# Kyaw-Thiha/animal-vision

Hardware: AMD Instinct MI355X
Metric: megapixels/sec per-frame pipeline (higher is better)
Workload: dtype f16

## Files before the change

animal-vision_amd/csrc/mst_fused.hip:

```cpp
#include <hip/hip_fp16.h>

#include <cstdio>
#include <cstdlib>
#include <cstring>

#include "avx_internal.h"
#include "mst_common.h"
#include "mst_tile_order.h"

namespace {

typedef float float4_t __attribute__((ext_vector_type(4)));
#ifndef AVX_FFN32_GM2
#define AVX_FFN32_GM2 1
#endif
constexpr int kFT = 512;
constexpr int TS = 16;
constexpr int HS = TS + 2;
#ifndef AVX_FFN_TH
#define AVX_FFN_TH 16
#endif
constexpr int kFfnTH = AVX_FFN_TH;
static_assert(kFfnTH == 14 || kFfnTH == 16, "FeedForward tile rows");
constexpr int kFfnNGRP = (HS * (kFfnTH + 2) + 31) / 32;

__device__ __forceinline__ float16_t mfma16(half8_t a, half8_t b, float16_t c) { return __builtin_amdgcn_mfma_f32_32x32x16_f16(a, b, c, 0, 0, 0); }

struct Tile { int x0, y0; long b; };
template <class Walk>
__device__ __forceinline__ Tile tile_at(const Walk& wk, int side_x, int side_y) { return Tile{wk.xi * side_x, wk.yi * side_y, (long)wk.b}; }
int mst_tile_order() {
    const char* e = getenv("AVX_MST_TILE_ORDER");
    return e && !strcmp(e, "raster") ? AVX_TILE_ORDER_RASTER : AVX_TILE_ORDER_XCD;
}

typedef _Float16 half16_t __attribute__((ext_vector_type(16)));
template <bool DWS>
__device__ __forceinline__ float4_t dw_unit(const half8_t (&a)[3], const uint4 (&bq)[3]) {
    float4_t acc = {0.f, 0.f, 0.f, 0.f};
    if constexpr (DWS) {
        const half8_t b0 = __builtin_bit_cast(half8_t, bq[0]), b1 = __builtin_bit_cast(half8_t, bq[1]);
        acc = __builtin_amdgcn_mfma_f32_16x16x32_f16(a[1], __builtin_bit_cast(half8_t, bq[2]), acc, 0, 0, 0);
        acc = __builtin_amdgcn_smfmac_f32_16x16x64_f16(a[0], __builtin_shufflevector(b0, b1, 0, 1, 2, 3, 4, 5, 6, 7, 8, 9, 10, 11, 12, 13, 14, 15), acc,
                                                       (int)__builtin_bit_cast(uint4, a[2]).x, 0, 0);
    } else {
#pragma unroll
        for (int i = 0; i < 3; ++i) acc = __builtin_amdgcn_mfma_f32_16x16x32_f16(a[i], __builtin_bit_cast(half8_t, bq[i]), acc, 0, 0, 0);
    }
    return acc;
}
template <bool DWS>
__device__ __forceinline__ half8_t dw_frag(const uint4* p, int i) {
    if (DWS && i == 2) return __builtin_bit_cast(half8_t, uint4{*reinterpret_cast<const unsigned*>(p), 0u, 0u, 0u});
    return __builtin_bit_cast(half8_t, *p);
}
template <bool MARCH> struct FfnWalk { typedef TileWalk type; };
template <> struct FfnWalk<true> { typedef ColumnWalk type; };
template <int C, int HPASS, int MINW, bool DWM, bool STAMP = false, int NW = 8, bool DWS = false, bool MARCH = false>
__global__ __launch_bounds__(64 * NW, MINW) void k_mst_ffn_fused(const __half* __restrict__ x , const float* __restrict__ gamma, const float* __restrict__ beta,
                                                          float eps, const uint4* __restrict__ w1pack , const __half* __restrict__ taps ,
                                                          const uint4* __restrict__ w2pack , __half* __restrict__ out , int B,
                                                          int H, int W, const uint4* __restrict__ dwpack , unsigned long long* __restrict__ stamps , int order ) {
    constexpr int FTH = MARCH ? 14 : kFfnTH, HSY = FTH + 2, ROW0 = MARCH ? 2 : 0, NHALO = HS * (HSY - ROW0), NGRP = (NHALO + 31) / 32;
    constexpr int HID = 4 * C, NPASS = HID / HPASS, KS1 = C / 16, KS2 = HPASS / 16, NT = C / 32, YPITCH = C * 2 + 16, LNV = C / 16;
    constexpr int HPITCH = HPASS * 2 + 16, RPITCH = (HS * HPITCH + 255) / 256 * 256 , NCT = HPASS / 32;
    static_assert(C == 32 || C == 64 || C == 128, "31-, 62- or 124-channel blocks (stored 32 / 64 / 128 wide)");
    constexpr int NTHR = 64 * NW, NGW = (NGRP + NW - 1) / NW;
    constexpr int NTW = NT / (NW / 8), NOCTW = HPASS / (8 * NW);
    static_assert((NW == 8 || NW == 16) && NT % (NW / 8) == 0 && (!DWM || HPASS % (8 * NW) == 0) && (DWM || NW == 8) && (DWM || !DWS) && (DWM || !MARCH), "wave split");
    constexpr bool PREFETCH = C <= 64;
    extern __shared__ __align__(16) unsigned char smem[];
    unsigned char* yt = smem;
    unsigned char* ht = yt + (size_t)NGRP * 32 * YPITCH;
    __half* tapl = reinterpret_cast<__half*>(ht + (size_t)HSY * RPITCH);
    float* gl = reinterpret_cast<float*>(tapl + (DWM ? 0 : 9 * HID));
    constexpr bool W2LDS = NW == 16;
    uint4* w2l = reinterpret_cast<uint4*>(gl + 2 * C);
    constexpr int NPRIME = 2 * HS, CARRY = NPRIME * HPITCH;
    unsigned char* carry = reinterpret_cast<unsigned char*>(w2l + (W2LDS ? NT * KS2 * 64 : 0));
    const int tid = threadIdx.x, lane = tid & 63, wave = tid >> 6, p = lane & 31, h = lane >> 5;
    unsigned long long seg[8] = {0, 0, 0, 0, 0, 0, 0, 0}, tlast = 0;
// ... 131 lines not shown
                    const float bq = is_pad(i + 1) ? 0.f : __builtin_fmaf(d[i + 1] * rstd, gl[c + 1], gl[C + c + 1]);
                    o[j / 2] = pack_f16(a, bq);
                }
                *reinterpret_cast<uint4*>(dst + 16 * v) = uint4{o[0], o[1], o[2], o[3]};
            }
        }
    };

    const int n0 = (wave / 8) * NTW, w8 = wave % 8;
    half8_t w2f[W2LDS ? 1 : NTW * KS2];
    auto load_w2 = [&](int pass) {
#pragma unroll
        for (int n = 0; n < NTW; ++n)
#pragma unroll
            for (int s = 0; s < KS2; ++s) w2f[n * KS2 + s] = __builtin_bit_cast(half8_t, w2pack[((size_t)(n0 + n) * (HID / 16) + pass * KS2 + s) * 64 + lane]);
    };
    if constexpr (NPASS == 1 && !W2LDS) load_w2(0);
    half8_t w1f[KS1];
    auto load_w1 = [&](int pass) {
#pragma unroll
        for (int s = 0; s < KS1; ++s) w1f[s] = __builtin_bit_cast(half8_t, w1pack[((size_t)(pass * NCT + wave % NCT) * KS1 + s) * 64 + lane]);
    };
    constexpr bool W1AHEAD = DWM && C == 64 && NPASS > 1 && NW == 8;
    static_assert(!(MARCH && W1AHEAD), "the marching form loads W1 at the top of phase 1 (priming replaces the fragments)");
    if constexpr (W1AHEAD) load_w1(0);
    constexpr int NITEM = (NGRP + NW / NCT - 1) / (NW / NCT);
    int p1_g[NITEM], p1_dst[NITEM], p1_dy[NITEM], p1_dx[NITEM];
#pragma unroll
    for (int j = 0; j < NITEM; ++j) {
        const int g = wave / NCT + j * (NW / NCT), q = 32 * g + p, qc = q < NHALO ? q : 0;
        p1_g[j] = g < NGRP ? g : -1;
        p1_dst[j] = (g < NGRP && q < NHALO) ? (ROW0 + qc / HS) * RPITCH + (qc % HS) * HPITCH + 32 * h : -1;
        p1_dy[j] = ROW0 + qc / HS - 1; p1_dx[j] = qc % HS - 1;
    }
    auto p1_item = [&](int g, unsigned char* base, int off, bool masked, int yy, int xx) {
        float16_t d;
#pragma unroll
        for (int v = 0; v < 16; ++v) d[v] = 0.f;
        const unsigned char* ysrc = yt + (size_t)(32 * g + p) * YPITCH + 16 * h;
#pragma unroll
        for (int s = 0; s < KS1; ++s) d = mfma16(w1f[s], __builtin_bit_cast(half8_t, *reinterpret_cast<const uint4*>(ysrc + 32 * s)), d);
        if (off >= 0) {
            unsigned char* dst = base + off;
            uint32_t keep = 0xffffffffu;
            if (masked) keep = (yy >= 0 && yy < H && xx >= 0 && xx < W) ? 0xffffffffu : 0u;
            constexpr int GP1 = (C == 64 && NW == 8) ? 4 : (C == 32 ? 2 : 1);
            unsigned pk[8];
#pragma unroll
// ... 19 lines not shown
        int td = tid;
        asm volatile("" : "+v"(td));
        const int wl = td >> 6, q = 32 * (wl / NCT) + (td & 31), qc = q < NPRIME ? q : 0, yy = t.y0 - 1 + qc / HS, xx = t.x0 - 1 + qc % HS;
        const int off = q < NPRIME ? qc * HPITCH + 32 * ((td >> 5) & 1) + 64 * (wl % NCT) : -1;
        if (g < NGPRIME) {
#pragma unroll 1
            for (int pass = 0; pass < NPASS; ++pass) {
                load_w1(pass);
                p1_item(g, carry + (size_t)pass * CARRY, off, true, yy, xx);
            }
        }
        __syncthreads();
    };
    typename FfnWalk<MARCH>::type ahead;
    if constexpr (MARCH) ahead.init(blockIdx.x, gridDim.x, B, ty, tx);
    else ahead.init(blockIdx.x, gridDim.x, B, ty, tx, order);
    if (!ahead.live) return;
    Tile t = tile_at(ahead, TS, FTH);
    ahead.advance();
    if constexpr (MARCH) prime(t);
    fetch(t);
    __syncthreads();
    layernorm(NGRP);
    for (;;) {
        const bool halo_inside = t.y0 + ROW0 >= 1 && t.y0 + HSY - 1 <= H && t.x0 >= 1 && t.x0 + HS - 1 <= W;
        float16_t D[NTW];
#pragma unroll
        for (int n = 0; n < NTW; ++n)
#pragma unroll
            for (int v = 0; v < 16; ++v) D[n][v] = 0.f;
#pragma unroll 1
        for (int pass = 0; pass < NPASS; ++pass) {
            stamp(pass == 0 ? 7 : 5);
            __syncthreads();
            stamp(0);
            if constexpr (W2LDS)
                for (int i = tid; i < NT * KS2 * 64; i += NTHR) w2l[i] = w2pack[((size_t)(i / (KS2 * 64)) * (HID / 16) + pass * KS2 + (i / 64) % KS2) * 64 + (i & 63)];
            half8_t af[DWM ? NOCTW : 1][3];
            if constexpr (DWM) {
#pragma unroll
                for (int o2 = 0; o2 < NOCTW; ++o2)
#pragma unroll
                    for (int i = 0; i < 3; ++i) af[o2][i] = dw_frag<DWS>(dwpack + ((size_t)(pass * (HPASS / 8) + NW * o2 + wave) * 3 + i) * 64 + lane, i);
            }
            {
                const int ct = wave % NCT;
                if constexpr (!W1AHEAD) load_w1(pass);
                if constexpr (MARCH) {
                    constexpr int NV = NPRIME * (HPASS / 8);
                    static_assert(NV <= NTHR, "one 16-byte piece per thread");
                    int i = tid;
                    asm volatile("" : "+v"(i));
                    if (i < NV) {
                        const int px = i / (HPASS / 8), o = i % (HPASS / 8);
                        *reinterpret_cast<uint4*>(ht + (size_t)(px / HS) * RPITCH + (size_t)(px % HS) * HPITCH + 16 * o) =
                            *reinterpret_cast<const uint4*>(carry + (size_t)pass * CARRY + (size_t)px * HPITCH + 16 * o);
                    }
                }
#pragma unroll
                for (int j = 0; j < NITEM; ++j) {
                    if (p1_g[j] < 0) continue;
                    p1_item(p1_g[j], ht + 64 * ct, p1_dst[j], !halo_inside, t.y0 + p1_dy[j], t.x0 + p1_dx[j]);
                }
            }
            stamp(1);
            __syncthreads();
            stamp(2);
            bool ahead_fetch = ahead.live;
            if constexpr (MARCH) ahead_fetch = ahead_fetch && !ahead.seg;
            if (PREFETCH && pass == NPASS - 1 && ahead_fetch) fetch(tile_at(ahead, TS, FTH));
// ... 93 lines not shown
#pragma unroll
                    for (int j = 0; j < 8; ++j) acc[j] = 0.f;
#pragma unroll
                    for (int tap = 0; tap < 9; ++tap) {
                        const uint4 hv = *reinterpret_cast<const uint4*>(hbase + (size_t)(tap / 3) * RPITCH + (size_t)(tap % 3) * HPITCH + 32 * s);
                        const uint4 wv = *reinterpret_cast<const uint4*>(tbase + (size_t)tap * HID * 2 + 32 * s);
                        fma_mix_lo(acc[0], hv.x, wv.x); fma_mix_hi(acc[1], hv.x, wv.x);
                        fma_mix_lo(acc[2], hv.y, wv.y); fma_mix_hi(acc[3], hv.y, wv.y);
                        fma_mix_lo(acc[4], hv.z, wv.z); fma_mix_hi(acc[5], hv.z, wv.z);
                        fma_mix_lo(acc[6], hv.w, wv.w); fma_mix_hi(acc[7], hv.w, wv.w);
                    }
                    half8_t bf;
#pragma unroll
                    for (int j = 0; j < 8; j += 2) {
                        const float2_t gv = gelu_fast2(float2_t{acc[j], acc[j + 1]});
                        bf[j] = (_Float16)gv.x;
                        bf[j + 1] = (_Float16)gv.y;
                    }
#pragma unroll
                    for (int n = 0; n < NT; ++n)
                        D[n] = mfma16(w2f[n * KS2 + s], bf, D[n]);
                }
            }
        }
        stamp(5);
        {
            const int yo = t.y0 + 2 * w8 + (p >> 4), xo = t.x0 + (p & 15);
            if (2 * w8 < FTH && yo < H && xo < W) {
                const size_t off = ((t.b * H + yo) * (size_t)W + xo) * C + 16 * h + 32 * n0;
#pragma unroll
                for (int n = 0; n < NTW; ++n) {
                    const uint4 xa = reinterpret_cast<const uint4*>(x + off + 32 * n)[0], xb = reinterpret_cast<const uint4*>(x + off + 32 * n)[1];
                    const unsigned xw[8] = {xa.x, xa.y, xa.z, xa.w, xb.x, xb.y, xb.z, xb.w};
                    unsigned ow[8];
#pragma unroll
                    for (int j = 0; j < 8; ++j) {
                        float s0 = D[n][2 * j], s1 = D[n][2 * j + 1];
                        fma_mix_lo(s0, xw[j], 0x3c003c00u); fma_mix_hi(s1, xw[j], 0x3c003c00u);
                        ow[j] = pack_f16(s0, s1);
                    }
                    reinterpret_cast<uint4*>(out + off + 32 * n)[0] = uint4{ow[0], ow[1], ow[2], ow[3]};
                    reinterpret_cast<uint4*>(out + off + 32 * n)[1] = uint4{ow[4], ow[5], ow[6], ow[7]};
                }
            }
        }
        stamp(6);
        if (!ahead.live) break;
        t = tile_at(ahead, TS, FTH);
        bool fetch_now = !PREFETCH;
        if constexpr (MARCH) {
            if (ahead.seg) { prime(t); fetch_now = true; }
        }
        ahead.advance();
        if (fetch_now) fetch(t);
        layernorm(NGRP);
    }
    if constexpr (STAMP) {
        if (lane == 0 && stamps)
#pragma unroll
            for (int k = 0; k < 8; ++k) stamps[((size_t)blockIdx.x * NW + wave) * 8 + k] = seg[k];
    }
}


constexpr int VS = TS + 4, MS = TS + 2;

template <int C, int MINW>
__global__ __launch_bounds__(kFT, MINW) void k_mst_attn_tail(const __half* __restrict__ v , const __half* __restrict__ x ,
                                                             const uint4* __restrict__ mpack , const __half* __restrict__ taps1 ,
                                                             const __half* __restrict__ taps2 , const float* __restrict__ bias ,
                                                             __half* __restrict__ out, int B, int H, int W, const uint4* __restrict__ wvpack ) {
    constexpr int NO = C / 8, NS = C / 16, NT = C / 32, PP = C * 2 + 16;
    constexpr int VRP = (VS * PP + 255) / 256 * 256, MRP = VRP;
    constexpr int NFILL = (VS * VS * NO + kFT - 1) / kFT;
    extern __shared__ __align__(16) unsigned char smem[];
    unsigned char* vt = smem;
    unsigned char* mt = vt + (size_t)VS * VRP;
    const bool fromx = wvpack != nullptr;
// ... 828 lines not shown
}
__device__ __forceinline__ void conv_in_mfma(const unsigned raw[5], half8_t a0, half8_t a1, uint4 o[2]) {
    const float inv255 = 1.0f / 255.0f;
    float v[16];
    v[15] = 0.f;
#pragma unroll
    for (int t = 0; t < 5; ++t)
#pragma unroll
        for (int c = 0; c < 3; ++c) v[3 * t + c] = (float)((raw[t] >> (8 * c)) & 0xffu) * inv255;
    const half8_t b0 = __builtin_bit_cast(half8_t, uint4{pack_f16(v[0], v[1]), pack_f16(v[2], v[3]), pack_f16(v[4], v[5]), pack_f16(v[6], v[7])});
    const half8_t b1 = __builtin_bit_cast(half8_t, uint4{pack_f16(v[8], v[9]), pack_f16(v[10], v[11]), pack_f16(v[12], v[13]), pack_f16(v[14], v[15])});
    float16_t d;
#pragma unroll
    for (int vv = 0; vv < 16; ++vv) d[vv] = 0.f;
    d = mfma16(a0, b0, d);
    d = mfma16(a1, b1, d);
    unsigned q[8];
#pragma unroll
    for (int vv = 0; vv < 8; ++vv) q[vv] = pack_f16(d[2 * vv], d[2 * vv + 1]);
    o[0] = uint4{q[0], q[1], q[2], q[3]};
    o[1] = uint4{q[4], q[5], q[6], q[7]};
}

template <int MINW, bool GRAM, bool SPEC = false, bool CINR = false, bool CINX = false>
__global__ __launch_bounds__(kFT, MINW) void k_mst_conv3x3_lds(const __half* __restrict__ x , const uint4* __restrict__ wpack ,
                                                               const __half* __restrict__ add , __half* __restrict__ out, int B, int H, int W,
                                                               const uint4* __restrict__ wqk , float* __restrict__ partial ,
                                                               const float* __restrict__ specw = nullptr ,
                                                               float* __restrict__ planes = nullptr , SpecStat3* __restrict__ spart = nullptr ,
                                                               int crop_t = 0, int crop_l = 0, int Hc = 0, int Wc = 0, int order = AVX_TILE_ORDER_RASTER ,
                                                               ConvInFrame cf = ConvInFrame{nullptr, 0, 0, 0, 0, 0, 0} , const float* __restrict__ cw = nullptr ) {
    static_assert(!(CINR && CINX), "the frame stands in for the residual or for the input");
    constexpr bool CIN = CINR || CINX;
    constexpr int C = 32, PP = C * 2 + 16, RP = (HS * PP + 255) / 256 * 256, NFILL = CINX ? 1 : (HS * HS * 4 + kFT - 1) / kFT;
    constexpr int SS = HS + 2;
    __shared__ __align__(16) unsigned char xt[HS * RP];
    __shared__ uint4 wl[18 * 64];
    __shared__ uint4 cwl[CIN ? 2 * 64 : 1];
    __shared__ unsigned st[CINX ? SS * SS : 1];
    const int tid = threadIdx.x, lane = tid & 63, wave = tid >> 6, p = lane & 31, h = lane >> 5;
    for (int i = tid; i < 18 * 64; i += kFT) wl[i] = wpack[i];
    if constexpr (CIN) {
        if (tid < 2 * 64) cwl[tid] = __builtin_bit_cast(uint4, conv_in_afrag(cw, lane, wave));
    }
    __shared__ uint4 wq[GRAM ? 4 * 64 : 1];
    float16_t G;
    float nq = 0.f, nk = 0.f;
    if constexpr (GRAM) {
        if (tid < 4 * 64) wq[tid] = wqk[tid];
#pragma unroll
        for (int v = 0; v < 16; ++v) G[v] = 0.f;
    }
    float smn[3] = {3.4e38f, 3.4e38f, 3.4e38f}, smx[3] = {-3.4e38f, -3.4e38f, -3.4e38f};
    double ssum[3] = {0.0, 0.0, 0.0};
    const int tx = (W + TS - 1) / TS, ty = (H + TS - 1) / TS;
    uint4 pre[NFILL];
    unsigned f_rel[NFILL];
#pragma unroll
    for (int k = 0; k < NFILL; ++k) {
        const int it = tid + k * kFT, itc = it < HS * HS * 4 ? it : 0, q = itc >> 2, part = itc & 3;
        f_rel[k] = (unsigned)(((q / HS) * W + q % HS) * C + 8 * part) * 2u;
    }
    auto fetch = [&](const Tile& t) {
        int tq = tid;
// ... 117 lines not shown
                if (add) { ar[0] = reinterpret_cast<const uint4*>(add + off)[0]; ar[1] = reinterpret_cast<const uint4*>(add + off)[1]; }
            }
            float16_t d;
#pragma unroll
            for (int v = 0; v < 16; ++v) d[v] = 0.f;
            const unsigned char* src = xt + (size_t)r * RP + (size_t)c * PP + 16 * h;
#pragma unroll
            for (int tap = 0; tap < 9; ++tap)
#pragma unroll
                for (int s2 = 0; s2 < 2; ++s2)
                    d = mfma16(__builtin_bit_cast(half8_t, wl[(2 * tap + s2) * 64 + lane]), __builtin_bit_cast(half8_t, *reinterpret_cast<const uint4*>(src + (size_t)(tap / 3) * RP + (size_t)(tap % 3) * PP + 32 * s2)), d);
            half8_t o0, o1;
            {
                const half8_t r0 = __builtin_bit_cast(half8_t, ar[0]), r1 = __builtin_bit_cast(half8_t, ar[1]);
#pragma unroll
                for (int v = 0; v < 8; ++v) { o0[v] = (_Float16)(d[v] + (float)r0[v]); o1[v] = (_Float16)(d[8 + v] + (float)r1[v]); }
            }
            if constexpr (SPEC) {
                float a3[3] = {0.f, 0.f, 0.f};
                auto chain = [&]() {
#pragma unroll
                    for (int j = 0; j < 16; ++j) {
                        const float v = (float)(j < 8 ? o0[j] : o1[j - 8]);
                        const float* wb = specw + (16 * h + j) * 4;
#pragma unroll
                        for (int k = 0; k < 3; ++k) a3[k] = __builtin_fmaf(v, wb[k], a3[k]);
                    }
                };
                if (h == 0) chain();
#pragma unroll
                for (int k = 0; k < 3; ++k) { const float lo = __shfl_xor(a3[k], 32); a3[k] = h ? lo : a3[k]; }
                if (h == 1) chain();
                const int yc = yo - crop_t, xc = xo - crop_l;
                if (h == 1 && live && yc >= 0 && yc < Hc && xc >= 0 && xc < Wc) {
#pragma unroll
                    for (int k = 0; k < 3; ++k) {
                        planes[(size_t)k * Hc * Wc + (size_t)yc * Wc + xc] = a3[k];
                        smn[k] = fminf(smn[k], a3[k]); smx[k] = fmaxf(smx[k], a3[k]); ssum[k] += (double)a3[k];
                    }
                }
            } else if (live) {
                reinterpret_cast<uint4*>(out + off)[0] = __builtin_bit_cast(uint4, o0);
                reinterpret_cast<uint4*>(out + off)[1] = __builtin_bit_cast(uint4, o1);
            }
            if constexpr (GRAM) {
                if (!live) { o0 = half8_t{0, 0, 0, 0, 0, 0, 0, 0}; o1 = o0; }
                float16_t dq, dk;
// ... 374 lines not shown
                            const void* w2pack, void* out, int B, int H, int W, int C, void* stream, bool sparse, bool march, int max_workgroups) {
    AVX_REQUIRE(ctx, x && gamma && beta && w1pack && w2pack && out && B > 0 && H > 0 && W > 0, "avx_mst_ffn_fused: NULL pointer or empty tensor");
    AVX_REQUIRE(ctx, C == 32 || C == 64 || C == 128, "avx_mst_ffn_fused: C=%d (32, 64 or 128: 31-channel groups stored 32 wide)", C);
    AVX_REQUIRE(ctx, ((((uintptr_t)x | (uintptr_t)w1pack | (uintptr_t)w2pack | (uintptr_t)out | (uintptr_t)taps_9xhid)) & 15u) == 0,
                "avx_mst_ffn_fused: pointers must be 16-byte aligned");
    AVX_REQUIRE(ctx, x != out, "avx_mst_ffn_fused: neighbouring tiles read each other's halo: the output cannot be the input");
    AVX_HIP(ctx, hipSetDevice(ctx->device));
    hipStream_t s = avx_pick_stream(ctx, stream);
    const int fth = march ? 14 : kFfnTH;
    const long total = (long)B * ((H + fth - 1) / fth) * ((W + TS - 1) / TS);
    const char* hp = getenv("AVX_MST_FFN_HPASS");
    const bool small = C == 32 && (march || !(hp && atoi(hp) == 128));
    const int hpass = (small || C == 128) ? 64 : 128, hpitch = hpass * 2 + 16, rpitch = (HS * hpitch + 255) / 256 * 256;
    const long cap = (long)ctx->num_cus * (small ? 2 : 1);
    const bool nw16 = C == 64 && dwpack && (march || !(getenv("AVX_MST_FFN_NW") && atoi(getenv("AVX_MST_FFN_NW")) == 8));
    const size_t lds = (size_t)(march ? 8 : kFfnNGRP) * 32 * (C * 2 + 16) + (size_t)(fth + 2) * rpitch + (dwpack ? 0 : (size_t)9 * 4 * C * 2) + sizeof(float) * 2 * C +
                       (nw16 ? (size_t)(C / 32) * (hpass / 16) * 1024 : 0) + (march ? (size_t)(4 * C / hpass) * 2 * HS * hpitch : 0);
    AVX_REQUIRE(ctx, total <= 0x7fffffffl, "avx_mst_ffn_fused: 2^31 tiles or more");
    AVX_REQUIRE(ctx, !march || (dwpack && (C == 32 || C == 64)), "avx_mst_ffn_fused: the marching form is built for the matrix-pipe kernels at C = 32 and 64");
    long nwg = total < cap ? total : cap;
    if (max_workgroups > 0 && max_workgroups < nwg) nwg = max_workgroups;
    const dim3 grid((unsigned)nwg);
    const int order = mst_tile_order();
#define AVX_FFN1M(CV, HP, MW, DW, NWV, SP, MR)                                                                                                   \
    {                                                                                                                                            \
        auto k = k_mst_ffn_fused<CV, HP, MW, DW, false, NWV, SP, MR>;                                                                            \
        AVX_HIP(ctx, hipFuncSetAttribute((const void*)k, hipFuncAttributeMaxDynamicSharedMemorySize, (int)lds));                                 \
        hipLaunchKernelGGL(k, grid, dim3(64 * NWV), lds, s, (const __half*)x, gamma, beta, eps, (const uint4*)w1pack, (const __half*)taps_9xhid, \
                           (const uint4*)w2pack, (__half*)out, B, H, W, (const uint4*)dwpack, (unsigned long long*)nullptr, order);              \
    }
#define AVX_FFN1S(CV, HP, MW, DW, NWV, SP) AVX_FFN1M(CV, HP, MW, DW, NWV, SP, false)
#define AVX_FFN1(CV, HP, MW, DW, NWV) AVX_FFN1S(CV, HP, MW, DW, NWV, false)
#define AVX_FFN(CV, HP, MW) { if (dwpack && sparse) AVX_FFN1S(CV, HP, MW, true, 8, true) else if (dwpack) AVX_FFN1(CV, HP, MW, true, 8) else AVX_FFN1(CV, HP, MW, false, 8) }
    if (dwpack && getenv("AVX_FFN_STAMPS") && ((C == 32 && small) || C == 64 || C == 128)) {
        unsigned long long* d_st = nullptr;
        const int nwv = nw16 ? 16 : 8;
        const size_t n = (size_t)grid.x * nwv * 8;
        AVX_HIP(ctx, hipMalloc((void**)&d_st, n * sizeof(unsigned long long)));
#define AVX_FFN_ST2(CV, HP, MW, NWV, SP, MR)                                                                                                     \
    {                                                                                                                                            \
        auto k = k_mst_ffn_fused<CV, HP, MW, true, true, NWV, SP, MR>;                                                                           \
        AVX_HIP(ctx, hipFuncSetAttribute((const void*)k, hipFuncAttributeMaxDynamicSharedMemorySize, (int)lds));                                 \
        hipLaunchKernelGGL(k, grid, dim3(64 * NWV), lds, s, (const __half*)x, gamma, beta, eps, (const uint4*)w1pack, (const __half*)taps_9xhid, \
                           (const uint4*)w2pack, (__half*)out, B, H, W, (const uint4*)dwpack, d_st, order);                                      \
    }
#define AVX_FFN_ST1(CV, HP, MW, NWV, SP) AVX_FFN_ST2(CV, HP, MW, NWV, SP, false)
#define AVX_FFN_ST(CV, HP, MW, NWV) { if (sparse) AVX_FFN_ST1(CV, HP, MW, NWV, true) else AVX_FFN_ST1(CV, HP, MW, NWV, false) }
#define AVX_FFN_STM(CV, HP, MW, NWV) { if (sparse) AVX_FFN_ST2(CV, HP, MW, NWV, true, true) else AVX_FFN_ST2(CV, HP, MW, NWV, false, true) }
        if (march && C == 32) AVX_FFN_STM(32, 64, 4, 8) else if (march) AVX_FFN_STM(64, 128, 1, 16)
        else if (C == 32) AVX_FFN_ST(32, 64, 4, 8) else if (nw16) AVX_FFN_ST(64, 128, 1, 16) else if (C == 64) AVX_FFN_ST(64, 128, 2, 8) else AVX_FFN_ST(128, 64, 2, 8)
#undef AVX_FFN_STM
#undef AVX_FFN_ST
#undef AVX_FFN_ST1
#undef AVX_FFN_ST2
        AVX_HIP(ctx, hipStreamSynchronize(s));
        unsigned long long* h_st = (unsigned long long*)malloc(n * sizeof(unsigned long long));
        AVX_HIP(ctx, hipMemcpy(h_st, d_st, n * sizeof(unsigned long long), hipMemcpyDeviceToHost));
        double tot[8] = {0}, w0[8] = {0}, w7[8] = {0};
        for (size_t i = 0; i < n; ++i) { tot[i & 7] += (double)h_st[i]; if (((i >> 3) % nwv) == 0) w0[i & 7] += (double)h_st[i]; if (((i >> 3) % nwv) == (size_t)nwv - 1) w7[i & 7] += (double)h_st[i]; }
        double all = 0;
        for (int k2 = 0; k2 < 8; ++k2) all += tot[k2];
        fprintf(stderr, "[ffn stamps C=%d%s] %u blocks x %d waves, mean cycles per wave %.0f; share per segment (all waves | first wave | last wave): ", C, march ? " march" : "", grid.x, nwv, all / (grid.x * (double)nwv));
        const char* nm[8] = {"bar1", "phase1", "bar2", "phase2a", "bar3", "phase2b", "epilogue", "ln+fetch"};
        for (int k2 = 0; k2 < 8; ++k2) fprintf(stderr, "%s %.1f%% | %.1f%% | %.1f%%  ", nm[k2], 100 * tot[k2] / all, 100 * w0[k2] * nwv / all, 100 * w7[k2] * nwv / all);
        fprintf(stderr, "\n");
        free(h_st);
        (void)hipFree(d_st);
    } else if (march && C == 32 && sparse) AVX_FFN1M(32, 64, 4, true, 8, true, true)
    else if (march && C == 32) AVX_FFN1M(32, 64, 4, true, 8, false, true)
    else if (march && sparse) AVX_FFN1M(64, 128, 1, true, 16, true, true)
    else if (march) AVX_FFN1M(64, 128, 1, true, 16, false, true)
    else if (C == 32 && small) AVX_FFN(32, 64, 4) else if (C == 32) AVX_FFN(32, 128, 2)
    else if (nw16 && sparse) AVX_FFN1S(64, 128, 1, true, 16, true)
    else if (nw16) AVX_FFN1(64, 128, 1, true, 16)
    else if (C == 64) AVX_FFN(64, 128, 2) else AVX_FFN(128, 64, 2)
#undef AVX_FFN
#undef AVX_FFN1
#undef AVX_FFN1S
#undef AVX_FFN1M
    AVX_HIP(ctx, hipGetLastError());
    return AVX_OK;
}

extern "C" int avx_mst_attn_tail(avx_ctx* ctx, const void* v, const void* x, const void* mpack16, const void* taps1_9xc, const void* taps2_9xc, const float* bias,
                                 void* out, int B, int H, int W, int C, void* stream) {
    if (!ctx) return AVX_ERR_INVALID;
    AVX_REQUIRE(ctx, v && x && mpack16 && taps1_9xc && taps2_9xc && out && B > 0 && H > 0 && W > 0, "avx_mst_attn_tail: NULL pointer or empty tensor");
    AVX_REQUIRE(ctx, C == 32 || C == 64, "avx_mst_attn_tail: C=%d (32 or 64)", C);
    AVX_REQUIRE(ctx, ((((uintptr_t)v | (uintptr_t)x | (uintptr_t)mpack16 | (uintptr_t)out | (uintptr_t)taps1_9xc | (uintptr_t)taps2_9xc)) & 15u) == 0,
                "avx_mst_attn_tail: pointers must be 16-byte aligned");
    AVX_REQUIRE(ctx, v != out, "avx_mst_attn_tail: tiles read their neighbours' rows of v: the output cannot be v (it may be x)");
    AVX_HIP(ctx, hipSetDevice(ctx->device));
    hipStream_t s = avx_pick_stream(ctx, stream);
    if (C == 32) return launch_attn_tail<32, 4>(ctx, v, x, mpack16, taps1_9xc, taps2_9xc, bias, out, B, H, W, s, nullptr);
    return launch_attn_tail<64, 2>(ctx, v, x, mpack16, taps1_9xc, taps2_9xc, bias, out, B, H, W, s, nullptr);
}

extern "C" int avx_mst_attn_tail_x(avx_ctx* ctx, const void* x, const void* wvpack16, const void* mpack16, const void* taps1_9xc, const void* taps2_9xc,
                                   const float* bias, void* out, int B, int H, int W, int C, void* stream) {
// ... 99 lines not shown
}

extern "C" int avx_mst_conv3x3_lds_spectral(avx_ctx* ctx, const void* x, const void* wpack16, const void* add, int H, int W, int C, const float* weights_host, int crop_t,
                                            int crop_l, int Hc, int Wc, float* planes_out, void* partials_out, int* n_partials, void* stream) {
    if (!ctx) return AVX_ERR_INVALID;
    AVX_REQUIRE(ctx, x && wpack16 && weights_host && planes_out && partials_out && n_partials && H > 0 && W > 0, "avx_mst_conv3x3_lds_spectral: NULL pointer or empty tensor");
    AVX_REQUIRE(ctx, C == 32, "avx_mst_conv3x3_lds_spectral: C=%d (32: the 31-band cube as stored)", C);
    AVX_REQUIRE(ctx, crop_t >= 0 && crop_l >= 0 && Hc > 0 && Wc > 0 && crop_t + Hc <= H && crop_l + Wc <= W, "avx_mst_conv3x3_lds_spectral: the crop window must lie inside the frame");
    AVX_REQUIRE(ctx, ((((uintptr_t)x | (uintptr_t)wpack16 | (uintptr_t)add | (uintptr_t)partials_out)) & 15u) == 0, "avx_mst_conv3x3_lds_spectral: pointers must be 16-byte aligned");
    AVX_HIP(ctx, hipSetDevice(ctx->device));
    hipStream_t s = avx_pick_stream(ctx, stream);
    avx_ws* ws = avx_workspace(ctx, s);
    if (!ws) return AVX_ERR_NOMEM;
    float wT[32 * 4];
    for (int b = 0; b < 32; ++b)
        for (int k = 0; k < 4; ++k) wT[b * 4 + k] = k < 3 ? weights_host[(size_t)k * 32 + b] : 0.0f;
    float* dwT = nullptr;
    int rc = avx_const_upload(ctx, ws, 2, wT, sizeof(wT), s, (void**)&dwT);
    if (rc) return rc;
    const long total = (long)((H + TS - 1) / TS) * ((W + TS - 1) / TS);
    const long cap = (long)ctx->num_cus * 2;
    const long blocks = total < cap ? total : cap;
    *n_partials = (int)blocks;
    hipLaunchKernelGGL((k_mst_conv3x3_lds<4, false, true>), dim3((unsigned)blocks), dim3(kFT), 0, s, (const __half*)x, (const uint4*)wpack16, (const __half*)add, (__half*)nullptr, 1, H, W,
                       (const uint4*)nullptr, (float*)nullptr, (const float*)dwT, planes_out, (SpecStat3*)partials_out, crop_t, crop_l, Hc, Wc);
    AVX_HIP(ctx, hipGetLastError());
    return AVX_OK;
}

extern "C" int avx_mst_conv3x3_lds_gram(avx_ctx* ctx, const void* x, const void* wpack16, const void* add, void* out, int H, int W, int C, const void* wqk16, float* gram,
                                        float* nq, float* nk, void* stream) {
    if (!ctx) return AVX_ERR_INVALID;
    AVX_REQUIRE(ctx, x && wpack16 && out && wqk16 && gram && nq && nk && H > 0 && W > 0, "avx_mst_conv3x3_lds_gram: NULL pointer or empty tensor");
    AVX_REQUIRE(ctx, C == 32, "avx_mst_conv3x3_lds_gram: C=%d (32: the 31-channel full-resolution convs)", C);
    AVX_REQUIRE(ctx, ((((uintptr_t)x | (uintptr_t)wpack16 | (uintptr_t)add | (uintptr_t)out | (uintptr_t)wqk16)) & 15u) == 0, "avx_mst_conv3x3_lds_gram: pointers must be 16-byte aligned");
    AVX_REQUIRE(ctx, x != out, "avx_mst_conv3x3_lds_gram: in-place convolution is not possible");
    AVX_HIP(ctx, hipSetDevice(ctx->device));
    hipStream_t s = avx_pick_stream(ctx, stream);
    avx_ws* ws = avx_workspace(ctx, s);
    if (!ws) return AVX_ERR_NOMEM;
    const long total = (long)((H + TS - 1) / TS) * ((W + TS - 1) / TS);
    const long cap = (long)ctx->num_cus * 2;
    const long blocks = total < cap ? total : cap;
    int rc = avx_ensure_scratch(ctx, ws, sizeof(float) * (size_t)blocks * 34 * 32);
    if (rc) return rc;
    float* partial = (float*)ws->d_scratch;
    hipLaunchKernelGGL((k_mst_conv3x3_lds<4, true>), dim3((unsigned)blocks), dim3(kFT), 0, s, (const __half*)x, (const uint4*)wpack16, (const __half*)add, (__half*)out, 1, H, W,
                       (const uint4*)wqk16, partial);
// ... 58 lines not shown
                                                int pad_right, const float* w_27x32_dev, const float* weights_host, int crop_t, int crop_l, int Hc, int Wc, float* planes_out,
                                                void* partials_out, int* n_partials, void* stream) {
    if (!ctx) return AVX_ERR_INVALID;
    AVX_REQUIRE(ctx, x && wpack16 && weights_host && planes_out && partials_out && n_partials, "avx_mst_conv3x3_lds_spectral_cin: NULL pointer");
    ConvInFrame cf;
    int rc = conv_in_frame_check(ctx, "avx_mst_conv3x3_lds_spectral_cin", frame_hwc, H, W, pad_top, pad_bottom, pad_left, pad_right, w_27x32_dev, &cf);
    if (rc) return rc;
    AVX_REQUIRE(ctx, crop_t >= 0 && crop_l >= 0 && Hc > 0 && Wc > 0 && crop_t + Hc <= cf.Hp && crop_l + Wc <= cf.Wp, "avx_mst_conv3x3_lds_spectral_cin: the crop window must lie inside the padded frame");
    AVX_REQUIRE(ctx, ((((uintptr_t)x | (uintptr_t)wpack16 | (uintptr_t)partials_out)) & 15u) == 0, "avx_mst_conv3x3_lds_spectral_cin: pointers must be 16-byte aligned");
    AVX_HIP(ctx, hipSetDevice(ctx->device));
    hipStream_t s = avx_pick_stream(ctx, stream);
    avx_ws* ws = avx_workspace(ctx, s);
    if (!ws) return AVX_ERR_NOMEM;
    float wT[32 * 4];
    for (int b = 0; b < 32; ++b)
        for (int k = 0; k < 4; ++k) wT[b * 4 + k] = k < 3 ? weights_host[(size_t)k * 32 + b] : 0.0f;
    float* dwT = nullptr;
    rc = avx_const_upload(ctx, ws, 2, wT, sizeof(wT), s, (void**)&dwT);
    if (rc) return rc;
    const long total = (long)((cf.Hp + TS - 1) / TS) * ((cf.Wp + TS - 1) / TS);
    const long cap = (long)ctx->num_cus * 2;
    const long blocks = total < cap ? total : cap;
    *n_partials = (int)blocks;
    hipLaunchKernelGGL((k_mst_conv3x3_lds<4, false, true, true>), dim3((unsigned)blocks), dim3(kFT), 0, s, (const __half*)x, (const uint4*)wpack16, (const __half*)nullptr, (__half*)nullptr, 1,
                       cf.Hp, cf.Wp, (const uint4*)nullptr, (float*)nullptr, (const float*)dwT, planes_out, (SpecStat3*)partials_out, crop_t, crop_l, Hc, Wc, (int)AVX_TILE_ORDER_RASTER, cf,
                       w_27x32_dev);
    AVX_HIP(ctx, hipGetLastError());
    return AVX_OK;
}

extern "C" int avx_mst_conv3x3_lds_gram_cin(avx_ctx* ctx, const uint8_t* frame_hwc, int H, int W, int pad_top, int pad_bottom, int pad_left, int pad_right, const float* w_27x32_dev,
                                            const void* wpack16, void* out, const void* wqk16, float* gram, float* nq, float* nk, void* stream) {
    if (!ctx) return AVX_ERR_INVALID;
    AVX_REQUIRE(ctx, wpack16 && out && wqk16 && gram && nq && nk, "avx_mst_conv3x3_lds_gram_cin: NULL pointer");
    ConvInFrame cf;
    int rc = conv_in_frame_check(ctx, "avx_mst_conv3x3_lds_gram_cin", frame_hwc, H, W, pad_top, pad_bottom, pad_left, pad_right, w_27x32_dev, &cf);
    if (rc) return rc;
    AVX_REQUIRE(ctx, ((((uintptr_t)wpack16 | (uintptr_t)out | (uintptr_t)wqk16)) & 15u) == 0, "avx_mst_conv3x3_lds_gram_cin: pointers must be 16-byte aligned");
    AVX_HIP(ctx, hipSetDevice(ctx->device));
    hipStream_t s = avx_pick_stream(ctx, stream);
    avx_ws* ws = avx_workspace(ctx, s);
    if (!ws) return AVX_ERR_NOMEM;
    const long total = (long)((cf.Hp + TS - 1) / TS) * ((cf.Wp + TS - 1) / TS);
    const long cap = (long)ctx->num_cus * 2;
    const long blocks = total < cap ? total : cap;
    rc = avx_ensure_scratch(ctx, ws, sizeof(float) * (size_t)blocks * 34 * 32);
    if (rc) return rc;
// ... 30 lines not shown
```

animal-vision_amd/ml/mst_plus_plus.py:

```python
from __future__ import annotations

from typing import Dict, List

import torch
import torch.nn.functional as F

DIM = 31
PAD = 32


def padded(n: int) -> int:
    assert n % DIM == 0
    return n // DIM * PAD


def pad_index(n: int, device=None) -> torch.Tensor:
    i = torch.arange(n, device=device)
    return (i // DIM) * PAD + i % DIM


def pad_channels(t: torch.Tensor, dims) -> torch.Tensor:
    for d in dims:
        n = t.shape[d]
        shape = list(t.shape)
# ... 139 lines not shown
        self._upfuse = os.environ.get("AVX_MST_NO_UPFUSE", "") == ""
        self._tail = os.environ.get("AVX_MST_NO_TAIL", "") == ""
        self._tailx = os.environ.get("AVX_MST_NO_TAILX", "") == ""
        self._down = os.environ.get("AVX_MST_NO_DOWN4X4", "") == ""
        self._qkv16 = os.environ.get("AVX_MST_NO_QKV16", "") == ""
        self._convgram = os.environ.get("AVX_MST_NO_CONVGRAM", "") == ""
        self._ffn = os.environ.get("AVX_MST_NO_FFN_FUSED", "") == ""
        self._gelu_pre = None
        self._dwmx = os.environ.get("AVX_MST_NO_DW_MFMA", "") == ""
        self._dwsp = os.environ.get("AVX_MST_NO_DW_SPARSE", "") == ""
        self.DW_SPARSE_FFN_C = (32, 64, 128)
        self.DW_SPARSE_TAIL_C = (32, 64)
        self._specfuse = os.environ.get("AVX_MST_NO_SPEC_FUSE", "") == ""
        self._cinfuse = os.environ.get("AVX_MST_NO_CONV_IN_FUSE", "") == ""
        self.FFN_FUSED_C = tuple(int(v) for v in os.environ.get("AVX_MST_FFN_FUSED_C", "32,64,128").split(",") if v)
        self._ffn_march = os.environ.get("AVX_MST_NO_FFN_MARCH", "") == ""
        self.FFN_MARCH_C = (32, 64)
        self._tail_march = os.environ.get("AVX_MST_NO_TAIL_MARCH", "") == ""
        self.TAIL_MARCH_C = (32, 64)
        self._convt16 = os.environ.get("AVX_MST_NO_CONVT16", "") == ""
        self.CONVT16_C = (64, 128)
        self.CONVT16_GRAM_C = (128,)
        self._ctx = {}

    def ctx(self, device: torch.device):
        from ..runtime import get_context

        idx = device.index if device.index is not None else torch.cuda.current_device()
        c = get_context(idx)
        if c.device != idx:
            raise RuntimeError(f"libavx context is on device {c.device}, tensor on cuda:{idx} (one process per GPU)")
        return c

    @staticmethod
    def _dt(t: torch.Tensor) -> int:
        if t.dtype == torch.float32:
            return 0
        if t.dtype == torch.float16:
            return 1
        raise TypeError(f"csrc/mst.hip kernels take float32/float16, got {t.dtype}")

    def gram(self, qkv: torch.Tensor, heads: int):
        from .._lib import lib

        b, n, c3 = qkv.shape
        c = c3 // 3
# ... 837 lines not shown
```

Before: 470.8.

## Prefetch next-pass FFN weights, defer residual epilogue, cache spectral weights in LDS

Adds a load-ahead variant of the fused FFN kernel. It issues the next pass's W1 (and W2) weight fragments at the end of the current pass, and computes depthwise-fragment addresses with opaque offsets. For C<=64 it loads the residual early and delays the add/store until after the next tile's layernorm, so global latency overlaps compute. It also routes the C=128 depthwise path to this variant and caches the spectral projection weights in LDS in the conv3x3 spec kernel. The cost is extra register pressure and more template instantiations, all gated by the AVX_MST_NO_LOAD_AHEAD environment variable.

```diff
diff --git a/animal-vision_amd/csrc/mst_fused.hip b/animal-vision_amd/csrc/mst_fused.hip
--- a/animal-vision_amd/csrc/mst_fused.hip
+++ b/animal-vision_amd/csrc/mst_fused.hip
@@ -34,6 +34,20 @@
     return e && !strcmp(e, "raster") ? AVX_TILE_ORDER_RASTER : AVX_TILE_ORDER_XCD;
 }
 
+#ifndef AVX_FFN_W1_AHEAD
+#define AVX_FFN_W1_AHEAD 1
+#endif
+#ifndef AVX_FFN_RES_LATE
+#define AVX_FFN_RES_LATE 1
+#endif
+#ifndef AVX_SPEC_W_LDS
+#define AVX_SPEC_W_LDS 1
+#endif
+bool mst_load_ahead() {
+    const char* e = getenv("AVX_MST_NO_LOAD_AHEAD");
+    return !(e && *e && strcmp(e, "0"));
+}
+
 typedef _Float16 half16_t __attribute__((ext_vector_type(16)));
 template <bool DWS>
 __device__ __forceinline__ float4_t dw_unit(const half8_t (&a)[3], const uint4 (&bq)[3]) {
@@ -56,7 +70,7 @@
 }
 template <bool MARCH> struct FfnWalk { typedef TileWalk type; };
 template <> struct FfnWalk<true> { typedef ColumnWalk type; };
-template <int C, int HPASS, int MINW, bool DWM, bool STAMP = false, int NW = 8, bool DWS = false, bool MARCH = false>
+template <int C, int HPASS, int MINW, bool DWM, bool STAMP = false, int NW = 8, bool DWS = false, bool MARCH = false, bool LA = false>
 __global__ __launch_bounds__(64 * NW, MINW) void k_mst_ffn_fused(const __half* __restrict__ x , const float* __restrict__ gamma, const float* __restrict__ beta,
                                                           float eps, const uint4* __restrict__ w1pack , const __half* __restrict__ taps ,
                                                           const uint4* __restrict__ w2pack , __half* __restrict__ out , int B,
@@ -234,8 +248,31 @@
         for (int s = 0; s < KS1; ++s) w1f[s] = __builtin_bit_cast(half8_t, w1pack[((size_t)(pass * NCT + wave % NCT) * KS1 + s) * 64 + lane]);
     };
     constexpr bool W1AHEAD = DWM && C == 64 && NPASS > 1 && NW == 8;
-    static_assert(!(MARCH && W1AHEAD), "the marching form loads W1 at the top of phase 1 (priming replaces the fragments)");
+    constexpr bool W1NEXT = LA && AVX_FFN_W1_AHEAD && DWM && (C == 128 || AVX_FFN_W1_AHEAD > 1), RESLATE = LA && AVX_FFN_RES_LATE && DWM && C <= 64;
+    static_assert(!(W1NEXT && W1AHEAD) && !(MARCH && W1AHEAD), "one placement of the W1 loads (the marching form's priming replaces the fragments: W1NEXT requests pass 0's behind it)");
+    static_assert(!(W1NEXT && W2LDS) || NT * KS2 * 64 == NTHR, "one w2l value per thread");
     if constexpr (W1AHEAD) load_w1(0);
+    half8_t w2n = half8_t{0, 0, 0, 0, 0, 0, 0, 0};
+    auto load_next = [&](int pass) {
+        __builtin_amdgcn_sched_barrier(0);
+        int tq = tid;
+        asm volatile("" : "+v"(tq));
+        unsigned o = (unsigned)(((tq >> 6) % NCT) * KS1 * 64 + (tq & 63)) * 16u;
+        asm volatile("" : "+v"(o));
+        const char* base = reinterpret_cast<const char*>(w1pack + (size_t)pass * NCT * KS1 * 64) + o;
+#pragma unroll
+        for (int s = 0; s < KS1; ++s) w1f[s] = __builtin_bit_cast(half8_t, *reinterpret_cast<const uint4*>(base + 1024 * s));
+        if constexpr (W2LDS) {
+            unsigned o2 = (unsigned)(((tq / (KS2 * 64)) * (HID / 16) + (tq / 64) % KS2) * 64 + (tq & 63)) * 16u;
+            asm volatile("" : "+v"(o2));
+            w2n = __builtin_bit_cast(half8_t, *reinterpret_cast<const uint4*>(reinterpret_cast<const char*>(w2pack + (size_t)pass * KS2 * 64) + o2));
+        }
+    };
+    auto drop_next = [&]() {
+#pragma unroll
+        for (int s = 0; s < KS1; ++s) asm volatile("" : "=v"(w1f[s]));
+        if constexpr (W2LDS) asm volatile("" : "=v"(w2n));
+    };
     constexpr int NITEM = (NGRP + NW / NCT - 1) / (NW / NCT);
     int p1_g[NITEM], p1_dst[NITEM], p1_dy[NITEM], p1_dx[NITEM];
 #pragma unroll
@@ -301,6 +338,7 @@
     fetch(t);
     __syncthreads();
     layernorm(NGRP);
+    if constexpr (W1NEXT) load_next(0);
     for (;;) {
         const bool halo_inside = t.y0 + ROW0 >= 1 && t.y0 + HSY - 1 <= H && t.x0 >= 1 && t.x0 + HS - 1 <= W;
         float16_t D[NTW];
@@ -313,10 +351,21 @@
             stamp(pass == 0 ? 7 : 5);
             __syncthreads();
             stamp(0);
-            if constexpr (W2LDS)
+            if constexpr (W2LDS && W1NEXT) w2l[tid] = __builtin_bit_cast(uint4, w2n);
+            else if constexpr (W2LDS)
                 for (int i = tid; i < NT * KS2 * 64; i += NTHR) w2l[i] = w2pack[((size_t)(i / (KS2 * 64)) * (HID / 16) + pass * KS2 + (i / 64) % KS2) * 64 + (i & 63)];
             half8_t af[DWM ? NOCTW : 1][3];
-            if constexpr (DWM) {
+            if constexpr (DWM && LA) {
+                int tq = tid;
+                asm volatile("" : "+v"(tq));
+                unsigned o = (unsigned)((tq >> 6) * 3 * 64 + (tq & 63)) * 16u;
+                asm volatile("" : "+v"(o));
+                const char* base = reinterpret_cast<const char*>(dwpack + (size_t)pass * (HPASS / 8) * 3 * 64) + o;
+#pragma unroll
+                for (int o2 = 0; o2 < NOCTW; ++o2)
+#pragma unroll
+                    for (int i = 0; i < 3; ++i) af[o2][i] = dw_frag<DWS>(reinterpret_cast<const uint4*>(base + (size_t)((NW * o2 * 3 + i) * 64) * 16), i);
+            } else if constexpr (DWM) {
 #pragma unroll
                 for (int o2 = 0; o2 < NOCTW; ++o2)
 #pragma unroll
@@ -324,7 +373,7 @@
             }
             {
                 const int ct = wave % NCT;
-                if constexpr (!W1AHEAD) load_w1(pass);
+                if constexpr (!W1AHEAD && !W1NEXT) load_w1(pass);
                 if constexpr (MARCH) {
                     constexpr int NV = NPRIME * (HPASS / 8);
                     static_assert(NV <= NTHR, "one 16-byte piece per thread");
@@ -464,15 +513,36 @@
                         D[n] = mfma16(w2f[n * KS2 + s], bf, D[n]);
                 }
             }
+            if constexpr (W1NEXT) {
+                if (pass + 1 < NPASS) load_next(pass + 1);
+                else drop_next();
+            }
         }
         stamp(5);
-        {
-            const int yo = t.y0 + 2 * w8 + (p >> 4), xo = t.x0 + (p & 15);
-            if (2 * w8 < FTH && yo < H && xo < W) {
-                const size_t off = ((t.b * H + yo) * (size_t)W + xo) * C + 16 * h + 32 * n0;
+        const int yo = t.y0 + 2 * w8 + (p >> 4), xo = t.x0 + (p & 15);
+        const bool ep_live = 2 * w8 < FTH && yo < H && xo < W;
+        size_t off = 0;
+        uint4 xr[RESLATE ? NTW : 1][2];
+        const size_t ep_org = ((t.b * H + t.y0) * (size_t)W + t.x0) * C * 2u;
+        unsigned ep_o = 0u;
+        if constexpr (RESLATE) {
+            int tq = tid;
+            asm volatile("" : "+v"(tq));
+            ep_o = (unsigned)(((2 * ((tq >> 6) % 8) + ((tq >> 4) & 1)) * W + (tq & 15)) * C + 16 * ((tq >> 5) & 1) + 32 * ((tq >> 9) * NTW)) * 2u;
+            ep_o = ep_live ? ep_o : (unsigned)(32 * ((tq >> 9) * NTW)) * 2u;
+            asm volatile("" : "+v"(ep_o));
+            const char* src = reinterpret_cast<const char*>(x) + ep_org + ep_o;
+#pragma unroll
+            for (int n = 0; n < NTW; ++n) { xr[n][0] = reinterpret_cast<const uint4*>(src + 64 * n)[0]; xr[n][1] = reinterpret_cast<const uint4*>(src + 64 * n)[1]; }
+        }
+        auto add_store = [&]() {
+            if (ep_live) {
+                if constexpr (!RESLATE) off = ((t.b * H + yo) * (size_t)W + xo) * C + 16 * h + 32 * n0;
 #pragma unroll
                 for (int n = 0; n < NTW; ++n) {
-                    const uint4 xa = reinterpret_cast<const uint4*>(x + off + 32 * n)[0], xb = reinterpret_cast<const uint4*>(x + off + 32 * n)[1];
+                    uint4 xa, xb;
+                    if constexpr (RESLATE) { xa = xr[n][0]; xb = xr[n][1]; }
+                    else { xa = reinterpret_cast<const uint4*>(x + off + 32 * n)[0]; xb = reinterpret_cast<const uint4*>(x + off + 32 * n)[1]; }
                     const unsigned xw[8] = {xa.x, xa.y, xa.z, xa.w, xb.x, xb.y, xb.z, xb.w};
                     unsigned ow[8];
 #pragma unroll
@@ -481,14 +551,29 @@
                         fma_mix_lo(s0, xw[j], 0x3c003c00u); fma_mix_hi(s1, xw[j], 0x3c003c00u);
                         ow[j] = pack_f16(s0, s1);
                     }
-                    reinterpret_cast<uint4*>(out + off + 32 * n)[0] = uint4{ow[0], ow[1], ow[2], ow[3]};
-                    reinterpret_cast<uint4*>(out + off + 32 * n)[1] = uint4{ow[4], ow[5], ow[6], ow[7]};
-                }
-            }
-        }
+                    uint4* dst = reinterpret_cast<uint4*>(out + off + 32 * n);
+                    if constexpr (RESLATE) dst = reinterpret_cast<uint4*>(reinterpret_cast<char*>(out) + ep_org + ep_o + 64 * n);
+                    dst[0] = uint4{ow[0], ow[1], ow[2], ow[3]};
+                    dst[1] = uint4{ow[4], ow[5], ow[6], ow[7]};
+                }
+            }
+        };
+        bool ep_late = RESLATE && ahead.live;
+        if constexpr (MARCH) ep_late = ep_late && !ahead.seg;
+        if (!ep_late) add_store();
         stamp(6);
         if (!ahead.live) break;
         t = tile_at(ahead, TS, FTH);
+        if constexpr (RESLATE) {
+            static_assert(PREFETCH, "the steady step below fetches nothing");
+            if (ep_late) {
+                ahead.advance();
+                layernorm(NGRP);
+                if constexpr (W1NEXT) load_next(0);
+                add_store();
+                continue;
+            }
+        }
         bool fetch_now = !PREFETCH;
         if constexpr (MARCH) {
             if (ahead.seg) { prime(t); fetch_now = true; }
@@ -496,6 +581,7 @@
         ahead.advance();
         if (fetch_now) fetch(t);
         layernorm(NGRP);
+        if constexpr (W1NEXT) load_next(0);
     }
     if constexpr (STAMP) {
         if (lane == 0 && stamps)
@@ -1370,7 +1456,7 @@
     o[1] = uint4{q[4], q[5], q[6], q[7]};
 }
 
-template <int MINW, bool GRAM, bool SPEC = false, bool CINR = false, bool CINX = false>
+template <int MINW, bool GRAM, bool SPEC = false, bool CINR = false, bool CINX = false, bool SPWL = false>
 __global__ __launch_bounds__(kFT, MINW) void k_mst_conv3x3_lds(const __half* __restrict__ x , const uint4* __restrict__ wpack ,
                                                                const __half* __restrict__ add , __half* __restrict__ out, int B, int H, int W,
                                                                const uint4* __restrict__ wqk , float* __restrict__ partial ,
@@ -1386,8 +1472,13 @@
     __shared__ uint4 wl[18 * 64];
     __shared__ uint4 cwl[CIN ? 2 * 64 : 1];
     __shared__ unsigned st[CINX ? SS * SS : 1];
+    constexpr bool WLDS = SPEC && SPWL && AVX_SPEC_W_LDS;
+    __shared__ __align__(16) float spw[WLDS ? 32 * 4 : 4];
     const int tid = threadIdx.x, lane = tid & 63, wave = tid >> 6, p = lane & 31, h = lane >> 5;
     for (int i = tid; i < 18 * 64; i += kFT) wl[i] = wpack[i];
+    if constexpr (WLDS) {
+        if (tid < 32 * 4) spw[tid] = specw[tid];
+    }
     if constexpr (CIN) {
         if (tid < 2 * 64) cwl[tid] = __builtin_bit_cast(uint4, conv_in_afrag(cw, lane, wave));
     }
@@ -1551,7 +1642,7 @@
 #pragma unroll
                     for (int j = 0; j < 16; ++j) {
                         const float v = (float)(j < 8 ? o0[j] : o1[j - 8]);
-                        const float* wb = specw + (16 * h + j) * 4;
+                        const float* wb = (WLDS ? spw : specw) + (16 * h + j) * 4;
 #pragma unroll
                         for (int k = 0; k < 3; ++k) a3[k] = __builtin_fmaf(v, wb[k], a3[k]);
                     }
@@ -1972,9 +2063,12 @@
     if (max_workgroups > 0 && max_workgroups < nwg) nwg = max_workgroups;
     const dim3 grid((unsigned)nwg);
     const int order = mst_tile_order();
-#define AVX_FFN1M(CV, HP, MW, DW, NWV, SP, MR)                                                                                                   \
+    const bool la = mst_load_ahead();
+#define AVX_FFN1M(CV, HP, MW, DW, NWV, SP, MR) AVX_FFN1L(CV, HP, MW, DW, NWV, SP, MR, false)
+#define AVX_FFN1A(CV, HP, MW, NWV, SP, MR) { if (la) AVX_FFN1L(CV, HP, MW, true, NWV, SP, MR, true) else AVX_FFN1L(CV, HP, MW, true, NWV, SP, MR, false) }
+#define AVX_FFN1L(CV, HP, MW, DW, NWV, SP, MR, LAV)                                                                                              \
     {                                                                                                                                            \
-        auto k = k_mst_ffn_fused<CV, HP, MW, DW, false, NWV, SP, MR>;                                                                            \
+        auto k = k_mst_ffn_fused<CV, HP, MW, DW, false, NWV, SP, MR, LAV>;                                                                       \
         AVX_HIP(ctx, hipFuncSetAttribute((const void*)k, hipFuncAttributeMaxDynamicSharedMemorySize, (int)lds));                                 \
         hipLaunchKernelGGL(k, grid, dim3(64 * NWV), lds, s, (const __half*)x, gamma, beta, eps, (const uint4*)w1pack, (const __half*)taps_9xhid, \
                            (const uint4*)w2pack, (__half*)out, B, H, W, (const uint4*)dwpack, (unsigned long long*)nullptr, order);              \
@@ -1987,9 +2081,10 @@
         const int nwv = nw16 ? 16 : 8;
         const size_t n = (size_t)grid.x * nwv * 8;
         AVX_HIP(ctx, hipMalloc((void**)&d_st, n * sizeof(unsigned long long)));
-#define AVX_FFN_ST2(CV, HP, MW, NWV, SP, MR)                                                                                                     \
+#define AVX_FFN_ST2(CV, HP, MW, NWV, SP, MR) { if (la && (MR || CV == 128)) AVX_FFN_ST3(CV, HP, MW, NWV, SP, MR, (MR || CV == 128)) else AVX_FFN_ST3(CV, HP, MW, NWV, SP, MR, false) }
+#define AVX_FFN_ST3(CV, HP, MW, NWV, SP, MR, LAV)                                                                                                \
     {                                                                                                                                            \
-        auto k = k_mst_ffn_fused<CV, HP, MW, true, true, NWV, SP, MR>;                                                                           \
+        auto k = k_mst_ffn_fused<CV, HP, MW, true, true, NWV, SP, MR, LAV>;                                                                      \
         AVX_HIP(ctx, hipFuncSetAttribute((const void*)k, hipFuncAttributeMaxDynamicSharedMemorySize, (int)lds));                                 \
         hipLaunchKernelGGL(k, grid, dim3(64 * NWV), lds, s, (const __half*)x, gamma, beta, eps, (const uint4*)w1pack, (const __half*)taps_9xhid, \
                            (const uint4*)w2pack, (__half*)out, B, H, W, (const uint4*)dwpack, d_st, order);                                      \
@@ -2003,6 +2098,7 @@
 #undef AVX_FFN_ST
 #undef AVX_FFN_ST1
 #undef AVX_FFN_ST2
+#undef AVX_FFN_ST3
         AVX_HIP(ctx, hipStreamSynchronize(s));
         unsigned long long* h_st = (unsigned long long*)malloc(n * sizeof(unsigned long long));
         AVX_HIP(ctx, hipMemcpy(h_st, d_st, n * sizeof(unsigned long long), hipMemcpyDeviceToHost));
@@ -2016,15 +2112,20 @@
         fprintf(stderr, "\n");
         free(h_st);
         (void)hipFree(d_st);
-    } else if (march && C == 32 && sparse) AVX_FFN1M(32, 64, 4, true, 8, true, true)
-    else if (march && C == 32) AVX_FFN1M(32, 64, 4, true, 8, false, true)
-    else if (march && sparse) AVX_FFN1M(64, 128, 1, true, 16, true, true)
-    else if (march) AVX_FFN1M(64, 128, 1, true, 16, false, true)
+    } else if (march && C == 32 && sparse) AVX_FFN1A(32, 64, 4, 8, true, true)
+    else if (march && C == 32) AVX_FFN1A(32, 64, 4, 8, false, true)
+    else if (march && sparse) AVX_FFN1A(64, 128, 1, 16, true, true)
+    else if (march) AVX_FFN1A(64, 128, 1, 16, false, true)
     else if (C == 32 && small) AVX_FFN(32, 64, 4) else if (C == 32) AVX_FFN(32, 128, 2)
     else if (nw16 && sparse) AVX_FFN1S(64, 128, 1, true, 16, true)
     else if (nw16) AVX_FFN1(64, 128, 1, true, 16)
-    else if (C == 64) AVX_FFN(64, 128, 2) else AVX_FFN(128, 64, 2)
+    else if (C == 64) AVX_FFN(64, 128, 2)
+    else if (dwpack && sparse) AVX_FFN1A(128, 64, 2, 8, true, false)
+    else if (dwpack) AVX_FFN1A(128, 64, 2, 8, false, false)
+    else AVX_FFN(128, 64, 2)
 #undef AVX_FFN
+#undef AVX_FFN1A
+#undef AVX_FFN1L
 #undef AVX_FFN1
 #undef AVX_FFN1S
 #undef AVX_FFN1M
@@ -2170,8 +2271,10 @@
     const long cap = (long)ctx->num_cus * 2;
     const long blocks = total < cap ? total : cap;
     *n_partials = (int)blocks;
-    hipLaunchKernelGGL((k_mst_conv3x3_lds<4, false, true>), dim3((unsigned)blocks), dim3(kFT), 0, s, (const __half*)x, (const uint4*)wpack16, (const __half*)add, (__half*)nullptr, 1, H, W,
-                       (const uint4*)nullptr, (float*)nullptr, (const float*)dwT, planes_out, (SpecStat3*)partials_out, crop_t, crop_l, Hc, Wc);
+    auto k = mst_load_ahead() ? k_mst_conv3x3_lds<4, false, true, false, false, true> : k_mst_conv3x3_lds<4, false, true>;
+    hipLaunchKernelGGL(k, dim3((unsigned)blocks), dim3(kFT), 0, s, (const __half*)x, (const uint4*)wpack16, (const __half*)add, (__half*)nullptr, 1, H, W,
+                       (const uint4*)nullptr, (float*)nullptr, (const float*)dwT, planes_out, (SpecStat3*)partials_out, crop_t, crop_l, Hc, Wc, (int)AVX_TILE_ORDER_RASTER,
+                       ConvInFrame{nullptr, 0, 0, 0, 0, 0, 0}, (const float*)nullptr);
     AVX_HIP(ctx, hipGetLastError());
     return AVX_OK;
 }
@@ -2276,7 +2379,8 @@
     const long cap = (long)ctx->num_cus * 2;
     const long blocks = total < cap ? total : cap;
     *n_partials = (int)blocks;
-    hipLaunchKernelGGL((k_mst_conv3x3_lds<4, false, true, true>), dim3((unsigned)blocks), dim3(kFT), 0, s, (const __half*)x, (const uint4*)wpack16, (const __half*)nullptr, (__half*)nullptr, 1,
+    auto k = mst_load_ahead() ? k_mst_conv3x3_lds<4, false, true, true, false, true> : k_mst_conv3x3_lds<4, false, true, true>;
+    hipLaunchKernelGGL(k, dim3((unsigned)blocks), dim3(kFT), 0, s, (const __half*)x, (const uint4*)wpack16, (const __half*)nullptr, (__half*)nullptr, 1,
                        cf.Hp, cf.Wp, (const uint4*)nullptr, (float*)nullptr, (const float*)dwT, planes_out, (SpecStat3*)partials_out, crop_t, crop_l, Hc, Wc, (int)AVX_TILE_ORDER_RASTER, cf,
                        w_27x32_dev);
     AVX_HIP(ctx, hipGetLastError());
diff --git a/animal-vision_amd/ml/mst_plus_plus.py b/animal-vision_amd/ml/mst_plus_plus.py
--- a/animal-vision_amd/ml/mst_plus_plus.py
+++ b/animal-vision_amd/ml/mst_plus_plus.py
@@ -185,6 +185,21 @@
         self.CONVT16_C = (64, 128)
         self.CONVT16_GRAM_C = (128,)
         self._ctx = {}
+
+    @property
+    def _load_ahead(self) -> bool:
+        import os
+
+        return os.environ.get("AVX_MST_NO_LOAD_AHEAD", "") in ("", "0")
+
+    @_load_ahead.setter
+    def _load_ahead(self, on: bool) -> None:
+        import os
+
+        if on:
+            os.environ.pop("AVX_MST_NO_LOAD_AHEAD", None)
+        else:
+            os.environ["AVX_MST_NO_LOAD_AHEAD"] = "1"
 
     def ctx(self, device: torch.device):
         from ..runtime import get_context
```

New measurement: 474.8, median of 6. About the same (+0.8%).
